# sleveque/control

Measured on NVIDIA B200. Metric: kkt_solve_time, lower is better.
Workload: dtype f64

## Files before the change

### control_b200/_lib.py

```python
import ctypes as C
import os

_HERE = os.path.dirname(os.path.abspath(__file__))
LIB_PATH = os.path.join(_HERE, "lib", "libctl_b200.so")

CTL_LAYOUT_BLOCK_MAJOR, CTL_LAYOUT_TIME_FASTEST = 0, 1
CTL_MAT_M, CTL_MAT_K, CTL_MAT_KT = 0, 1, 2
CTL_KSP_GMRES, CTL_KSP_FGMRES, CTL_KSP_MINRES = 0, 1, 2
CTL_PC_NONE, CTL_PC_BUILTIN, CTL_PC_CALLBACK = 0, 1, 2
CTL_PCMODE_TRIANGULAR, CTL_PCMODE_DIAGONAL = 0, 1
CTL_S0_JACOBI, CTL_S0_CHEBYSHEV, CTL_S0_AMG = 0, 1, 2
CTL_HISTORY_MAX = 1024


class ctl_config(C.Structure):
    _fields_ = [("n", C.c_int32), ("n_t", C.c_int32), ("CN", C.c_int32), ("device", C.c_int32),
                ("tau", C.c_double), ("beta", C.c_double), ("epsilon", C.c_double),
                ("stream", C.c_void_p), ("rank", C.c_int32), ("world", C.c_int32)]


class ctl_pc_options(C.Structure):
    _fields_ = [("mode", C.c_int32), ("solver_0", C.c_int32),
                ("cheb_emin", C.c_double), ("cheb_emax", C.c_double),
                ("cheb_steps", C.c_int32), ("amg_cycles", C.c_int32), ("amg_nu", C.c_int32),
                ("amg_nu_fine", C.c_int32),
                ("amg_max_levels", C.c_int32), ("amg_coarse_max", C.c_int32),
                ("amg_theta", C.c_double), ("amg_lo", C.c_double), ("amg_hi", C.c_double),
                ("amg_acc_lo", C.c_double), ("amg_acc_hi", C.c_double)]


class ctl_krylov_options(C.Structure):
    _fields_ = [("ksp_type", C.c_int32), ("restart", C.c_int32), ("max_it", C.c_int32),
                ("pc", C.c_int32), ("rtol", C.c_double), ("atol", C.c_double),
                ("divtol", C.c_double)]


class ctl_solve_result(C.Structure):
    _fields_ = [("its", C.c_int32), ("reason", C.c_int32), ("n_mult", C.c_int32),
                ("n_pc", C.c_int32), ("rnorm", C.c_double), ("ref_norm", C.c_double),
                ("n_history", C.c_int32), ("history", C.c_double * CTL_HISTORY_MAX),
                ("seconds_total", C.c_double), ("seconds_mult", C.c_double),
                ("seconds_pc", C.c_double)]

# ... 20 lines not shown
    "ctl_set_pattern": (C.c_int, [_H, C.c_void_p, C.c_void_p, C.c_int64]),
    "ctl_set_values": (C.c_int, [_H, C.c_int, C.c_int, C.c_void_p]),
    "ctl_set_bc": (C.c_int, [_H, C.c_void_p, C.c_int32]),
    "ctl_set_block_size": (C.c_int, [_H, C.c_int32]),
    "ctl_assemble": (C.c_int, [_H]),
    "ctl_n_blocks": (C.c_int32, [_H]),
    "ctl_ld": (C.c_int32, [_H]),
    "ctl_n_local": (C.c_int32, [_H]),
    "ctl_row_begin": (C.c_int32, [_H]),
    "ctl_vec_len": (C.c_int64, [_H, C.c_int]),
    "ctl_convert_layout": (C.c_int, [_H, _F64P, C.c_int, _F64P, C.c_int]),
    "ctl_kkt_apply": (C.c_int, [_H, _F64P, _F64P, C.c_int]),
    "ctl_pc_default_options": (C.c_int, [C.POINTER(ctl_pc_options)]),
    "ctl_pc_setup": (C.c_int, [_H, C.POINTER(ctl_pc_options)]),
    "ctl_pc_block_size": (C.c_int32, [_H]),
    "ctl_pc_apply": (C.c_int, [_H, _F64P, _F64P, C.c_int]),
    "ctl_pc_fn": (C.c_int, [_H, _F64P, _F64P, C.c_int]),
    "ctl_set_pc_callback": (C.c_int, [_H, PC_CALLBACK, C.c_void_p]),
    "ctl_krylov_default_options": (C.c_int, [C.POINTER(ctl_krylov_options)]),
    "ctl_solve": (C.c_int, [_H, _F64P, _F64P, C.c_int, C.POINTER(ctl_krylov_options),
                            C.POINTER(ctl_solve_result)]),
    "ctl_solve_host": (C.c_int, [_H, _F64P, _F64P, C.POINTER(ctl_krylov_options),
                                 C.POINTER(ctl_solve_result)]),
    "ctl_kkt_residual_norm": (C.c_int, [_H, _F64P, _F64P, C.c_int, C.POINTER(C.c_double)]),
    "ctl_nonlinear_residual": (C.c_int, [_H, _F64P, _F64P, _F64P, C.c_int, C.POINTER(C.c_double)]),
    "ctl_objective_host": (C.c_int, [_H, _F64P, _F64P, _F64P, C.POINTER(C.c_double)]),
    "ctl_objective": (C.c_int, [_H, _F64P, _F64P, _F64P, C.POINTER(C.c_double)]),
    "ctl_build_rhs": (C.c_int, [_H, _F64P, _F64P, _F64P, _F64P]),
    "ctl_lift_bc": (C.c_int, [_H, _F64P, _F64P, C.c_int]),
    "ctl_amg_num_hierarchies": (C.c_int32, [_H]),
# ... 60 lines not shown
```

### control_b200/csrc/amg.cu

```cuda
#include "amg.cuh"

#include <cstdlib>
#include <stdexcept>

#include "cheb_coefficients.h"

int amg_build_distributed(ctl_handle_s *h, const AmgParams &p, const std::shared_ptr<SellPattern> &fine_pattern,
                          AmgHierarchyDev &H);

static int dev_alloc(ctl_handle_s *h, double **p, size_t n)
{
    CTL_CUDA(cudaMalloc((void **)p, std::max<size_t>(n, 1) * sizeof(double)));
    CTL_CUDA(cudaMemsetAsync(*p, 0, std::max<size_t>(n, 1) * sizeof(double), h->stream));
    return CTL_OK;
}

int amg_level_vectors(ctl_handle_s *h, AmgLevelDev &L, int level)
{
    const size_t nv = (size_t)L.n * L.A.nc;
    CTL_TRY(dev_alloc(h, &L.r, nv));
    CTL_TRY(dev_alloc(h, &L.t0, nv));
    CTL_TRY(dev_alloc(h, &L.t1, nv));
    CTL_TRY(dev_alloc(h, &L.t2, nv));
    if (level > 0) {
// ... 10 lines not shown
    const int64_t nc = H.nc;
    int64_t bytes = 0;
    for (int l = 0; l < nl; ++l) {
        const AmgLevelDev &L = H.dev[l];
        if (l + 1 < nl) {
            const int nu_l = (l == 0 && p.nu_fine > 0) ? p.nu_fine : p.nu;
            bytes += (L.A.bytes_per_pass + (8ll + 32ll * nc) * L.n) * (2 * nu_l);
            bytes += L.P.bytes_per_pass + L.R.bytes_per_pass + 32ll * nc * L.n;
        } else if (L.Ainv) {
            bytes += 8ll * L.n * L.n;
        } else {
            bytes += (L.A.bytes_per_pass + (8ll + 32ll * nc) * L.n) * p.nu;
        }
    }
    return bytes;
}

int amg_build(ctl_handle_s *h, const HostCSR &A0, const AmgParams &p,
              const std::shared_ptr<SellPattern> &fine_pattern, AmgHierarchyDev &H)
{
    H.params = p;
    try {
        if (H.host.empty()) amg_setup_host(A0, p, H.host);
    } catch (const std::exception &e) {
        ctl_set_error(h, e.what());
        return CTL_ERR_STATE;
    }
    const int nl = (int)H.host.size();
    H.dev.assign(nl, AmgLevelDev());
    CTL_CHECK(H.nc == 1 || h->cfg.world == 1, CTL_ERR_ARG, "amg_build: block hierarchies run on one GPU only");
// ... 11 lines not shown
            Ld.A.nc = H.nc;
            CTL_TRY(ctl_upload(h, &Ld.dinv, Lh.dinv.data(), (size_t)Ld.n));
            CTL_TRY(amg_level_vectors(h, Ld, l));
            if (l + 1 < nl) {
                CTL_TRY(sell_from_csr(h, Lh.P, Ld.P));
                CTL_TRY(sell_from_csr(h, Lh.R, Ld.R));
                Ld.P.nc = Ld.R.nc = H.nc;
            } else if (!Lh.Ainv.empty()) {
                CTL_TRY(dense_inverse_upload(h, Lh.Ainv, Ld.n, &Ld.Ainv, &Ld.Ainv_ld));
            } else if (Lh.coarse_inverse) {
                CTL_TRY(dense_inverse_device(h, Lh.A, Lh.coarse_shift, &Ld.Ainv, &Ld.Ainv_ld));
            }
        }
    }
    H.bytes_per_cycle = amg_cycle_bytes(H);
    if (p.acc_lo > 0.0) {
        const size_t nv = (size_t)H.dev[0].n * H.nc;
        CTL_TRY(dev_alloc(h, &H.acc_r, nv));
        CTL_TRY(dev_alloc(h, &H.acc_z, nv));
        CTL_TRY(dev_alloc(h, &H.acc_p, nv));
    }
    return CTL_OK;
}

void amg_free(AmgHierarchyDev &H)
{
    cudaFree(H.acc_r);
    cudaFree(H.acc_z);
    cudaFree(H.acc_p);
    H.acc_r = H.acc_z = H.acc_p = nullptr;
// ... 103 lines not shown

namespace {
__global__ void lincomb3_kernel(double *out, double a, const double *x, double b, const double *__restrict__ y,
                                double c, const double *__restrict__ z, int n)
{
    pdl_sync();
    const int i = blockIdx.x * blockDim.x + threadIdx.x;
    if (i >= n) return;
    double r = c * z[i];
    if (y) r = fma(b, y[i], r);
    if (x) r = fma(a, x[i], r);
    out[i] = r;
}
}

int amg_solve(ctl_handle_s *h, AmgHierarchyDev &H, const double *b, double *x, bool b_exchanged)
{
    const AmgParams &p = H.params;
    AmgLevelDev &L0 = H.dev[0];
    if (L0.pb && !b_exchanged) CTL_TRY(halo_exchange_now(h, L0.pb, b));
    const GVec gb = L0.pb ? GVec(b, halo_ll(L0.pb), halo_idx1(L0.pb)) : GVec(b);
    if (p.acc_lo <= 0.0) {
        for (int c = 0; c < p.cycles; ++c) CTL_TRY(vcycle(h, H, 0, gb, x, c == 0));
        return CTL_OK;
    }
    CTL_CHECK(!L0.px, CTL_ERR_STATE, "amg_solve: accelerated cycles are not available on several GPUs");
    const int n = L0.n * H.nc;
    double scale;
    std::vector<double> om;
    cheb_coefficients(p.acc_lo, p.acc_hi, p.cycles, &scale, om);
    double *buf[2] = {x, H.acc_p};
    auto slot = [&](int k) { return (p.cycles - k) & 1; };
    const int blocks = ceil_div(n, 256);
    CTL_TRY(vcycle(h, H, 0, gb, H.acc_z, true));
// ... 14 lines not shown
```

### control_b200/csrc/amg.cuh

```cuda
#pragma once
#include "amg_setup.h"
#include "sell.cuh"

struct AmgLevelDev {
    int n = 0;
    int n_ghost = 0;
    bool distributed = false;
    double rho = 0.0;
    SellMat A, P, R;
    double *dinv = nullptr;
    double *x = nullptr, *b = nullptr;
    double *r = nullptr, *t0 = nullptr, *t1 = nullptr, *t2 = nullptr;
    double *Ainv = nullptr;
    int Ainv_ld = 0;
    HaloPlan *px = nullptr, *pb = nullptr;
    HaloPlan *pr = nullptr;
    HaloPlan *prep = nullptr;
};

struct AmgHierarchyDev {
    AmgParams params;
    int nc = 1;
    std::vector<AmgLevelHost> host;
    std::vector<AmgLevelDev> dev;
    std::vector<std::shared_ptr<struct HaloSpace>> spaces;
    int64_t bytes_per_cycle = 0;
    double *acc_r = nullptr, *acc_z = nullptr, *acc_p = nullptr;
};

int amg_build(ctl_handle_s *h, const HostCSR &A0, const AmgParams &p,
              const std::shared_ptr<SellPattern> &fine_pattern, AmgHierarchyDev &H);
void amg_free(AmgHierarchyDev &H);
int dense_inverse_device(ctl_handle_s *h, const HostCSR &A, const std::vector<double> &shift, double **Ainv_out, int *lda_out);
int dense_inverse_upload(ctl_handle_s *h, const std::vector<double> &Ainv, int n, double **Ainv_out, int *lda_out);
int amg_solve(ctl_handle_s *h, AmgHierarchyDev &H, const double *b, double *x, bool b_exchanged = false);
```

### control_b200/csrc/amg_setup.h

```cpp
#pragma once
#include <vector>

#include "common.cuh"

enum { AMG_COARSE_INVERSE = 0,
       AMG_COARSE_PINV_CONSTANT = 1,
       AMG_COARSE_SMOOTH = 2 };

struct AmgParams {
    double theta = 0.08;
    double theta_decay = 0.5;
    int max_levels = 10;
    int coarse_max = 2500;
    int nu = 3;
    int nu_fine = 0;
    double lo = 0.25, hi = 1.0;
    int cycles = 3;
    double acc_lo = 0.0, acc_hi = 1.0;
    int coarse = 0;
    int device_inverse = 1;
};

struct AmgLevelHost {
    HostCSR A;
    std::vector<double> dinv;
    double rho = 0.0;
    std::vector<int> agg;
    HostCSR P, R;
    std::vector<double> Ainv;
    int coarse_inverse = 0;
    std::vector<double> coarse_shift;
    bool has_inverse() const { return !Ainv.empty() || coarse_inverse != 0; }
};

// ... 5 lines not shown
```

### control_b200/csrc/pc.cu

```cuda
#include "pc.cuh"

#include <atomic>
#include <chrono>
#include <cstdio>
#include <map>
#include <cmath>
#include <cstdlib>
#include <cstring>
#include <thread>

#include "cheb_coefficients.h"
#include "vec_ops.cuh"

namespace {

void combine_global(ctl_handle_s *h, int level, bool transposed, double w, double m_coef, bool identity,
                    std::vector<double> &out)
{
    const std::vector<int> &ip = h->h_indptr, &ix = h->h_indices;
    const int lv = h->h_K.size() > 1 ? level : 0;
    const std::vector<double> &Kv = h->h_K[lv];
    const std::vector<double> *KTv = h->h_KT.empty() ? nullptr : &h->h_KT[lv];
    out.assign(ix.size(), 0.0);
    for (int r = 0; r < h->n; ++r) {
// ... 291 lines not shown
    o->mode = CTL_PCMODE_TRIANGULAR;
    o->solver_0 = CTL_S0_JACOBI;
    o->cheb_emin = 0.0;
    o->cheb_emax = 0.0;
    o->cheb_steps = 20;
    o->amg_cycles = d.cycles;
    o->amg_nu = d.nu;
    o->amg_nu_fine = d.nu_fine;
    o->amg_max_levels = d.max_levels;
    o->amg_coarse_max = d.coarse_max;
    o->amg_theta = d.theta;
    o->amg_lo = d.lo;
    o->amg_hi = d.hi;
    o->amg_acc_lo = d.acc_lo;
    o->amg_acc_hi = d.acc_hi;
    return CTL_OK;
}

int ctl_amg_setup_probe(const int32_t *indptr, const int32_t *indices, const double *values, int32_t n,
                        const ctl_pc_options *opts, int32_t *n_levels, int32_t *level_n, int64_t *level_nnz,
                        double *level_rho, int32_t *aggregates)
{
    if (!indptr || !indices || !values || n <= 0 || !n_levels) return CTL_ERR_ARG;
    AmgParams p;
    if (opts) {
        p.theta = opts->amg_theta;
        p.max_levels = opts->amg_max_levels;
        p.coarse_max = opts->amg_coarse_max;
        p.nu = opts->amg_nu;
        p.nu_fine = opts->amg_nu_fine;
// ... 46 lines not shown
{
    SetupLap lap;
    CTL_CHECK(h && opts, CTL_ERR_ARG, "ctl_pc_setup: null argument");
    CTL_CHECK(h->assembled, CTL_ERR_STATE, "ctl_pc_setup: ctl_assemble has not been called");
    CTL_CHECK(opts->mode == CTL_PCMODE_TRIANGULAR || opts->mode == CTL_PCMODE_DIAGONAL, CTL_ERR_ARG,
              "ctl_pc_setup: unknown mode");
    CTL_CHECK(opts->solver_0 >= CTL_S0_JACOBI && opts->solver_0 <= CTL_S0_AMG, CTL_ERR_ARG,
              "ctl_pc_setup: unknown solver_0");
    if (opts->solver_0 == CTL_S0_CHEBYSHEV)
        CTL_CHECK(opts->cheb_emax > opts->cheb_emin && opts->cheb_emin > 0 && opts->cheb_steps >= 1, CTL_ERR_ARG,
                  "ctl_pc_setup: Chebyshev needs 0 < e_min < e_max and at least one step");
    CTL_CHECK(opts->amg_cycles >= 1 && opts->amg_nu >= 1 && opts->amg_nu_fine >= 0 && opts->amg_max_levels >= 1,
              CTL_ERR_ARG, "ctl_pc_setup: bad AMG options");
    CTL_CHECK(opts->amg_acc_lo <= 0.0 || opts->amg_acc_hi > opts->amg_acc_lo, CTL_ERR_ARG,
              "ctl_pc_setup: AMG acceleration needs acc_lo < acc_hi");
    if (opts->mode == CTL_PCMODE_DIAGONAL)
        CTL_CHECK(h->cfg.CN && !h->per_level && h->k_symmetric, CTL_ERR_ARG,
                  "ctl_pc_setup: the block-diagonal (MINRES) variant needs CN and a time-independent symmetric K");
    CTL_CHECK(h->cfg.world == 1 || h->comm, CTL_ERR_STATE, "ctl_pc_setup: call ctl_comm_init first (world > 1)");
    CTL_CUDA(cudaSetDevice(h->cfg.device));
    ctl_pc_free(h);
    h->pc = std::make_shared<PcState>();
    PcState &st = *h->pc;
    st.opts = *opts;
    st.amg.theta = opts->amg_theta;
    st.amg.max_levels = opts->amg_max_levels;
    st.amg.coarse_max = opts->amg_coarse_max;
    st.amg.nu = opts->amg_nu;
    st.amg.nu_fine = opts->amg_nu_fine;
    st.amg.lo = opts->amg_lo;
    st.amg.hi = opts->amg_hi;
    st.amg.cycles = opts->amg_cycles;
    st.amg.acc_lo = opts->amg_acc_lo;
    st.amg.acc_hi = opts->amg_acc_hi;
    if (const char *e = getenv("CTL_NO_GRAPH")) st.use_graph = !(e[0] == '1');

    const int N = h->N, nl = h->n_loc, rb = h->row_begin;
    const bool cn = h->cfg.CN != 0;
    const double tau = h->cfg.tau, beta = h->cfg.beta, eps = h->cfg.epsilon;
    if (h->h_KT.empty() && !h->k_symmetric && h->h_tperm.size() != h->h_indices.size()) {
        const std::vector<int> &ip = h->h_indptr, &ix = h->h_indices;
        h->h_tperm.resize(ix.size());
        for (int r = 0; r < h->n; ++r)
            for (int k = ip[r]; k < ip[r + 1]; ++k) {
                const int c = ix[k];
                const int *b = ix.data() + ip[c], *e = ix.data() + ip[c + 1];
                h->h_tperm[k] = (int)(std::lower_bound(b, e, r) - ix.data());
            }
    }
// ... 251 lines not shown
    std::copy(A.indptr.begin(), A.indptr.end(), indptr);
    std::copy(A.indices.begin(), A.indices.end(), indices);
    std::copy(A.values.begin(), A.values.end(), values);
    return CTL_OK;
}

int ctl_amg_get_aggregates(ctl_handle h, int32_t hi, int32_t lvl, int32_t *agg)
{
    AMG_LEVEL(h, hi, lvl);
    std::copy(L.agg.begin(), L.agg.end(), agg);
    return CTL_OK;
}

int32_t ctl_pc_block_size(ctl_handle h) { return (h && h->pc && h->pc->ready) ? h->pc->bs : -1; }

int ctl_amg_solve(ctl_handle h, int32_t hi, const double *b, double *x)
{
    CTL_CHECK(h && h->pc && hi >= 0 && hi < (int)h->pc->hier.size() && b && x, CTL_ERR_ARG, "ctl_amg_solve: bad argument");
    CTL_CHECK(h->pc->hier[hi].nc != 2 || (((uintptr_t)b | (uintptr_t)x) & 15) == 0, CTL_ERR_ARG,
              "ctl_amg_solve: a block-size-2 hierarchy needs 16-byte aligned vectors");
    CTL_CUDA(cudaSetDevice(h->cfg.device));
    CTL_TRY(halo_epoch_begin(h));
    CTL_TRY(amg_solve(h, h->pc->hier[hi], b, x, false));
    return ctl_comm_check(h);
}

int ctl_time_amg(ctl_handle h, int32_t hi, int reps, int flush_l2, double *out)
{
    CTL_CHECK(h && h->pc && hi >= 0 && hi < (int)h->pc->hier.size() && out && reps > 0, CTL_ERR_ARG,
              "ctl_time_amg: bad argument");
// ... 73 lines not shown
```

### control_b200/csrc/sell.cu

```cuda
#include <algorithm>
#include <cstdlib>
#include <cstring>
#include <type_traits>

#include "sell.cuh"

SellPattern::~SellPattern()
{
    cudaFree(sp);
    cudaFree(cols);
    cudaFree(dcol);
}

void sell_free(SellMat &m)
{
    cudaFree(m.vals);
    cudaFree(m.vcode);
    cudaFree(m.vdict);
    cudaFree(m.code);
    cudaFree(m.dict);
    cudaFree(m.sp4);
    cudaFree(m.stab);
    cudaFree(m.csr_ptr);
    cudaFree(m.csr_cols);
// ... 298 lines not shown
    if constexpr (NC == 2) {
        *reinterpret_cast<double2 *>(out + 2 * row) = make_double2(v.c[0], v.c[1]);
    } else {
#pragma unroll
        for (int k = 0; k < NC; ++k) out[NC * row + k] = v.c[k];
    }
}
template <int NC>
__device__ __forceinline__ vec_t<NC> gat(const DVec &v, int c, unsigned seq_hi, const HaloCtx &ctx)
{
    if constexpr (NC == 1) return dvec_get(v, c, seq_hi, ctx);
    else return ld_node<NC>(v.x, c);
}

template <typename G, typename G0, typename PRE>
__device__ __forceinline__ auto sell_row_dot_stencil(const MatView &A, int row, G g, G0 g_own, PRE pre)
{
    const int s = row >> 5, lane = row & 31;
    const int4 s0 = pre_ld(A.sp4 + s);
    const int first = s << 5;
    const bool spec = A.ps_w > 0 && first + A.ps_dmin >= 0 && first + 31 + A.ps_dmax < A.n_own;
    pdl_wait();
    pre();
    using R = decltype(g(0));
    R acc{};
    if (spec) {
        R xv[8];
#pragma unroll
        for (int j = 0; j < 8; ++j) xv[j] = (j < A.ps_w) ? g_own(row + A.ps_delta[j]) : R{};
        if (s0.z == A.ps_off) {
#pragma unroll
            for (int j = 0; j < 8; ++j)
                if (j < A.ps_w) acc = vfma(A.ps_v[j], xv[j], acc);
            if (A.ps_w > 8) {
// ... 31 lines not shown
            for (int j = 0; j < SC; ++j) xv[j] = (k0 + j < s0.y) ? g(row + d[j]) : R{};
#pragma unroll
            for (int j = 0; j < SC; ++j)
                if (k0 + j < s0.y) acc = vfma(__ldg(&st[k0 + j].v), xv[j], acc);
        }
        return acc;
    }
    const int end = s0.x + 32 * s0.y;
    const uint16_t *code = reinterpret_cast<const uint16_t *>(A.code);
#pragma unroll 1
    for (int p = s0.x + lane; p < end; p += 32) {
        const DictEnt e = sf_dict(A.dict, __ldg(code + p));
        acc = vfma(e.v, g(row + e.delta), acc);
    }
    return acc;
}

template <int FMT, bool STREAM, typename G, typename G0, typename PRE>
__device__ __forceinline__ auto sell_row_dot(const MatView &A, int row, G g, G0 g_own, PRE pre)
{
    if (FMT == FMT_STENCIL) return sell_row_dot_stencil(A, row, g, g_own, pre);
    const int s = row >> 5, lane = row & 31;
    const int2 s0 = pre_ld(A.sp + s);
    const int end = pre_ld(reinterpret_cast<const int *>(A.sp + s + 1));
    using R = decltype(g(0));
    R acc{};
    auto chunk = [&](int p0, auto first) {
        constexpr bool PRE = decltype(first)::value;
        SfRaw raw[SC];
#pragma unroll
// ... 215 lines not shown
{
    const unsigned hi = kernel_prologue(ctx);
    run_rows<1, BS>(A.n_rows, push, hi, out, [&](int row) {
        const double di = pre_ld(dinv.x + row);
        vec_t<NC> bi{};
        const vec_t<NC> ax = sell_row_dot<FMT, STREAM>(
            A, row,
            [&](int c) {
                if constexpr (GH) return s * dvec_get(dinv, c, hi, ctx) * dvec_get(b, c, hi, ctx);
                else return s * __ldg(dinv.x + c) * ld_node<NC>(b.x, c);
            },
            [&](int c) { return s * __ldg(dinv.x + c) * ld_node<NC>(b.x, c); }, [&] { bi = ld_node<NC>(b.x, row); });
        const vec_t<NC> p1 = s * di * bi;
        return wgt * p1 + (wgt * s) * di * (bi - ax);
    });
}

template <int NC>
__global__ void __launch_bounds__(ST) sell_spmv2_kernel(const MatView A1, const MatView A2, const DVec x1, const DVec x2,
                                                       const DVec x3, double *y, double alpha, double beta,
                                                       const HaloCtx ctx, const HaloPush push)
{
    const unsigned hi = kernel_prologue(ctx);
    run_rows<1>(A1.n_rows, push, hi, y, [&](int row) {
        vec_t<NC> acc1;
        if (x2.x) acc1 = sell_row_dot_rt(A1, row, [&](int c) { return gat<NC>(x1, c, hi, ctx) + gat<NC>(x2, c, hi, ctx); });
        else acc1 = sell_row_dot_rt(A1, row, [&](int c) { return gat<NC>(x1, c, hi, ctx); });
        vec_t<NC> acc2{};
        if (x3.x) acc2 = sell_row_dot_rt(A2, row, [&](int c) { return gat<NC>(x3, c, hi, ctx); });
        return alpha * acc1 + beta * acc2;
// ... 333 lines not shown
    const DVec d1 = dvec(x1, V1), d2 = dvec(x2, V1), d3 = dvec(x3, V2);
    const HaloCtx ctx = halo_ctx(h);
    if (A1.nc == 2) pdl_launch(h, grid, ST, sell_spmv2_kernel<2>, V1, V2, d1, d2, d3, y, alpha, beta, ctx, push);
    else if (A1.nc == 3) pdl_launch(h, grid, ST, sell_spmv2_kernel<3>, V1, V2, d1, d2, d3, y, alpha, beta, ctx, push);
    else pdl_launch(h, grid, ST, sell_spmv2_kernel<1>, V1, V2, d1, d2, d3, y, alpha, beta, ctx, push);
    h->launches++;
    CTL_CUDA(cudaGetLastError());
    return CTL_OK;
}

int vec_copy_n(ctl_handle_s *h, double *dst, const double *src, int n)
{
    CTL_CUDA(cudaMemcpyAsync(dst, src, (size_t)n * sizeof(double), cudaMemcpyDeviceToDevice, h->stream));
    return CTL_OK;
}
```

### control_b200/csrc/sell.cuh

```cuda
#pragma once
#include <memory>

#include "common.cuh"
#include "halo.cuh"
#include "sell_format.h"

struct SellPattern {
    int n_rows = 0, n_cols = 0, n_slices = 0;
    int64_t n_stored = 0, nnz = 0;
    int2 *sp = nullptr;
    int *cols = nullptr;
    uint16_t *dcol = nullptr;
    SfSellLayout host;
    ~SellPattern();
};

struct SellMat {
    std::shared_ptr<SellPattern> pat;
    int fmt = FMT_F64;
    bool stream = false;
    int n_own = 0;
    int nc = 1;
    int64_t bytes_per_pass = 0;
    double *vals = nullptr;
// ... 42 lines not shown
};

int sell_spmv(ctl_handle_s *h, const SellMat &A, const GVec &x, double *y, const double *b, int mode,
              const HaloPush &push = HaloPush());
int sell_cheb_step(ctl_handle_s *h, const SellMat &A, const double *dinv, const double *b, const double *p_prev,
                   const GVec &p_cur, double *out, double a, double bq, double c, double prev_scale = 0.0,
                   const HaloPush &push = HaloPush());
int sell_cheb_first2(ctl_handle_s *h, const SellMat &A, const GVec &dinv, const GVec &b, double *out, double s, double w,
                     const HaloPush &push = HaloPush());
int vec_dinv_scale(ctl_handle_s *h, const double *dinv, const double *b, double *out, double c, int n,
                   const HaloPush &push = HaloPush(), int nc = 1);
int dense_gemv(ctl_handle_s *h, const double *Ainv, const double *b, double *y, int n, int lda, int nc = 1);
int sell_spmv2(ctl_handle_s *h, const SellMat &A1, const SellMat &A2, const GVec &x1, const GVec &x2, const GVec &x3,
               double *y, double alpha, double beta, const HaloPush &push = HaloPush());
int vec_copy_n(ctl_handle_s *h, double *dst, const double *src, int n);
```

### control_b200/system.py

```python
import ctypes as C

import numpy as np
import torch

from . import _lib as L

__all__ = ["MultiBlockSystem", "KSPInfo", "csr_arrays"]

_KSP_TYPES = {"gmres": L.CTL_KSP_GMRES, "fgmres": L.CTL_KSP_FGMRES, "minres": L.CTL_KSP_MINRES}

_error_flag = [False]


def csr_arrays(A):
    if isinstance(A, (tuple, list)) and len(A) == 3:
        indptr, indices, data = A
    else:
        A = A.tocsr()
        if not A.has_sorted_indices:
            A = A.sorted_indices()
        indptr, indices, data = A.indptr, A.indices, A.data
    return (np.ascontiguousarray(indptr, dtype=np.int32),
            np.ascontiguousarray(indices, dtype=np.int32),
            np.ascontiguousarray(data, dtype=np.float64))
# ... 203 lines not shown
        o = L.ctl_pc_options()
        self._check(self._lib.ctl_pc_default_options(C.byref(o)))
        o.mode = {"triangular": L.CTL_PCMODE_TRIANGULAR, "diagonal": L.CTL_PCMODE_DIAGONAL}[mode]
        if Multigrid:
            o.solver_0 = L.CTL_S0_AMG
        elif lambda_v_bounds is not None:
            o.solver_0 = L.CTL_S0_CHEBYSHEV
            o.cheb_emin, o.cheb_emax = float(lambda_v_bounds[0]), float(lambda_v_bounds[1])
        else:
            o.solver_0 = L.CTL_S0_JACOBI
        o.cheb_steps = int(cheb_steps)
        for key, field in (("cycles", "amg_cycles"), ("nu", "amg_nu"), ("nu_fine", "amg_nu_fine"),
                           ("max_levels", "amg_max_levels"),
                           ("coarse_max", "amg_coarse_max"), ("theta", "amg_theta"),
                           ("lo", "amg_lo"), ("hi", "amg_hi"), ("acc_lo", "amg_acc_lo"),
                           ("acc_hi", "amg_acc_hi")):
            if key in amg:
                setattr(o, field, amg.pop(key))
        if amg:
            raise TypeError(f"unknown AMG options {sorted(amg)}")
        self._check(self._lib.ctl_pc_setup(self._h, C.byref(o)))
        self._pc_ready = True
        self._pc_opts = o

    @property
    def pc_block_size(self):
        return int(self._lib.ctl_pc_block_size(self._h))

    def pc_apply(self, b_dev, u_dev=None, layout=L.CTL_LAYOUT_BLOCK_MAJOR, raw=False):
        if u_dev is None:
            u_dev = torch.zeros_like(b_dev)
        fn = self._lib.ctl_pc_fn if raw else self._lib.ctl_pc_apply
        self._call(fn, b_dev.data_ptr(), u_dev.data_ptr(), layout)
        return u_dev

    def pc_fn(self):
        def pc_fn(u_0, u_1, b_0, b_1):
            u = self.pc_apply(self.to_device(b_0, b_1), raw=True)
            r0, r1 = self.to_host_blocks(u)
            np.copyto(_as_host_f64(u_0).reshape(r0.shape), r0)
            np.copyto(_as_host_f64(u_1).reshape(r1.shape), r1)
        return pc_fn
# ... 271 lines not shown
```

### include/ctl_b200.h

```cpp
#ifndef CTL_B200_H
#define CTL_B200_H

#include <stdint.h>

#ifdef __cplusplus
extern "C" {
#endif

typedef struct ctl_handle_s *ctl_handle;

enum { CTL_OK = 0, CTL_ERR_ARG = -1, CTL_ERR_CUDA = -2, CTL_ERR_STATE = -3, CTL_ERR_NCCL = -4,
       CTL_ERR_CALLBACK = -5 };

enum { CTL_LAYOUT_BLOCK_MAJOR = 0, CTL_LAYOUT_TIME_FASTEST = 1 };

enum { CTL_MAT_M = 0, CTL_MAT_K = 1, CTL_MAT_KT = 2 };

enum { CTL_KSP_GMRES = 0, CTL_KSP_FGMRES = 1, CTL_KSP_MINRES = 2 };

enum { CTL_PC_NONE = 0,
       CTL_PC_BUILTIN = 1,
       CTL_PC_CALLBACK = 2 };

enum { CTL_PCMODE_TRIANGULAR = 0,
// ... 21 lines not shown
} ctl_config;

typedef struct {
    int32_t mode;
    int32_t solver_0;
    double cheb_emin, cheb_emax;
    int32_t cheb_steps;
    int32_t amg_cycles;
    int32_t amg_nu;
    int32_t amg_nu_fine;
    int32_t amg_max_levels;
    int32_t amg_coarse_max;
    double amg_theta;
    double amg_lo, amg_hi;
    double amg_acc_lo, amg_acc_hi;
} ctl_pc_options;

typedef struct {
    int32_t ksp_type;
    int32_t restart;
    int32_t max_it;
    int32_t pc;
    double rtol, atol;
    double divtol;
} ctl_krylov_options;

#define CTL_HISTORY_MAX 1024
typedef struct {
    int32_t its;
    int32_t reason;
// ... 21 lines not shown
int ctl_assemble(ctl_handle h);

int32_t ctl_n_blocks(ctl_handle h);
int32_t ctl_ld(ctl_handle h);
int32_t ctl_n_local(ctl_handle h);
int32_t ctl_row_begin(ctl_handle h);
int64_t ctl_vec_len(ctl_handle h, int layout);
int ctl_convert_layout(ctl_handle h, const double *src, int src_layout, double *dst,
                       int dst_layout);

int ctl_kkt_apply(ctl_handle h, const double *x, double *y, int layout);

int ctl_pc_default_options(ctl_pc_options *opts);
int ctl_pc_setup(ctl_handle h, const ctl_pc_options *opts);
int32_t ctl_pc_block_size(ctl_handle h);
int ctl_pc_apply(ctl_handle h, const double *b, double *u, int layout);
int ctl_pc_fn(ctl_handle h, const double *b, double *u, int layout);
int ctl_set_pc_callback(ctl_handle h, ctl_pc_callback fn, void *user);

int ctl_krylov_default_options(ctl_krylov_options *opts);
int ctl_solve(ctl_handle h, const double *b, double *u, int layout,
              const ctl_krylov_options *opts, ctl_solve_result *result);
int ctl_solve_host(ctl_handle h, const double *b_host, double *u_host,
                   const ctl_krylov_options *opts, ctl_solve_result *result);

int ctl_kkt_residual_norm(ctl_handle h, const double *b, const double *x, int layout,
                          double *out);
int ctl_nonlinear_residual(ctl_handle h, const double *b, const double *x, double *r, int layout,
                           double *norm_host);
int ctl_objective_host(ctl_handle h, const double *v_host, const double *zeta_host,
// ... 62 lines not shown
```

Measured before the change: 1.198.

## Fuse multiple fine-level Chebyshev smoothing steps into one shared-memory tiled kernel

Adds a temporal-blocking kernel that keeps a tile of the fine-level iterate plus a halo of k*band rows in shared memory and applies up to k Chebyshev/residual steps per launch. The plan derives band width and tile size from the stencil pattern, SM count and opt-in shared memory. The AMG solve switches to this fused path when conditions hold (single device, stencil format, single component, no acceleration), which is on by default (-1). The aim is fewer kernel launches and less global memory traffic per smoother sweep, at the cost of redundant halo computation and one block per SM.

```diff
diff --git a/control_b200/_lib.py b/control_b200/_lib.py
--- a/control_b200/_lib.py
+++ b/control_b200/_lib.py
@@ -26,7 +26,7 @@
                 ("amg_nu_fine", C.c_int32),
                 ("amg_max_levels", C.c_int32), ("amg_coarse_max", C.c_int32),
                 ("amg_theta", C.c_double), ("amg_lo", C.c_double), ("amg_hi", C.c_double),
-                ("amg_acc_lo", C.c_double), ("amg_acc_hi", C.c_double)]
+                ("amg_acc_lo", C.c_double), ("amg_acc_hi", C.c_double), ("amg_fine_fusion", C.c_int32)]
 
 
 class ctl_krylov_options(C.Structure):
@@ -77,6 +77,8 @@
     "ctl_pc_default_options": (C.c_int, [C.POINTER(ctl_pc_options)]),
     "ctl_pc_setup": (C.c_int, [_H, C.POINTER(ctl_pc_options)]),
     "ctl_pc_block_size": (C.c_int32, [_H]),
+    "ctl_pc_fine_fusion": (C.c_int32, [_H]),
+    "ctl_fine_fusion_plan": (C.c_int, [C.c_int32, C.c_int32, C.c_int32, C.c_int32, C.c_int32, _I32P]),
     "ctl_pc_apply": (C.c_int, [_H, _F64P, _F64P, C.c_int]),
     "ctl_pc_fn": (C.c_int, [_H, _F64P, _F64P, C.c_int]),
     "ctl_set_pc_callback": (C.c_int, [_H, PC_CALLBACK, C.c_void_p]),
diff --git a/control_b200/csrc/amg.cu b/control_b200/csrc/amg.cu
--- a/control_b200/csrc/amg.cu
+++ b/control_b200/csrc/amg.cu
@@ -48,6 +48,29 @@
         }
     }
     return bytes;
+}
+
+static int fine_fusion_setup(ctl_handle_s *h, AmgHierarchyDev &H)
+{
+    H.ff = FfPlan();
+    const AmgParams &p = H.params;
+    const int nu0 = p.nu_fine > 0 ? p.nu_fine : p.nu;
+    if (p.fine_fusion == 0 || h->cfg.world > 1 || H.nc != 1 || p.acc_lo > 0.0 || H.dev.size() < 2 || nu0 < 2) return CTL_OK;
+    const AmgLevelDev &L = H.dev[0];
+    if (L.A.lanes || L.A.fmt != FMT_STENCIL || L.px || L.pb) return CTL_OK;
+    const SfSellLayout &lay = L.A.pat->host;
+    int band = 0;
+    for (int s = 0; s < lay.n_slices; ++s)
+        for (int64_t q = lay.sp[s].x; q < lay.sp[s + 1].x; ++q) {
+            const int row = 32 * s + (int)((q - lay.sp[s].x) & 31);
+            if (row < L.n) band = std::max(band, std::abs(lay.cols[q] - row));
+        }
+    int dev = 0, n_sm = 0, smem = 0;
+    CTL_CUDA(cudaGetDevice(&dev));
+    CTL_CUDA(cudaDeviceGetAttribute(&n_sm, cudaDevAttrMultiProcessorCount, dev));
+    CTL_CUDA(cudaDeviceGetAttribute(&smem, cudaDevAttrMaxSharedMemoryPerBlockOptin, dev));
+    H.ff = fine_fusion_plan(L.n, band, n_sm, smem, p.fine_fusion > 0 ? p.fine_fusion : 0);
+    return sell_fused_prepare(h, H.ff);
 }
 
 int amg_build(ctl_handle_s *h, const HostCSR &A0, const AmgParams &p,
@@ -89,6 +112,7 @@
         }
     }
     H.bytes_per_cycle = amg_cycle_bytes(H);
+    CTL_TRY(fine_fusion_setup(h, H));
     if (p.acc_lo > 0.0) {
         const size_t nv = (size_t)H.dev[0].n * H.nc;
         CTL_TRY(dev_alloc(h, &H.acc_r, nv));
@@ -222,10 +246,102 @@
 }
 }
 
+static int amg_solve_fused(ctl_handle_s *h, AmgHierarchyDev &H, const double *b, double *x)
+{
+    const AmgParams &p = H.params;
+    AmgLevelDev &L = H.dev[0];
+    AmgLevelDev &C = H.dev[1];
+    const int nu = p.nu_fine > 0 ? p.nu_fine : p.nu;
+    double scale;
+    std::vector<double> om;
+    cheb_coefficients(p.lo * L.rho, p.hi * L.rho, nu, &scale, om);
+    auto step = [&](int k, bool zero) {
+        FfOp o;
+        o.kind = FF_CHEB;
+        if (k == 1) {
+            o.a = 0.0;
+            o.bq = 1.0;
+            o.c = scale;
+        } else {
+            const double w = om[k - 2];
+            o.a = 1.0 - w;
+            o.bq = w;
+            o.c = w * scale;
+            if (zero && k == 3) o.prev_scale = scale;
+        }
+        return o;
+    };
+    double *pool[5] = {x, L.t0, L.t1, L.t2, L.r};
+    auto run_chain = [&](const std::vector<FfOp> &ops, const double *cur_in, double **res) -> int {
+        const int k = H.ff.k, n_ops = (int)ops.size();
+        const double *in_cur = cur_in, *in_prev = nullptr;
+        for (int g0 = 0; g0 < n_ops; g0 += k) {
+            FfGroup g;
+            g.n_ops = std::min(k, n_ops - g0);
+            for (int j = 0; j < g.n_ops; ++j) g.op[j] = ops[g0 + j];
+            g.cur_in = in_cur;
+            g.prev_in = in_prev;
+            const bool final = g0 + g.n_ops == n_ops;
+            const FfOp &next = final ? ops[0] : ops[g0 + g.n_ops];
+            const bool need_prev = !final && next.kind == FF_CHEB && next.prev_scale == 0.0 && next.a != 0.0;
+            std::vector<double *> free_;
+            for (double *v : pool)
+                if (v != in_cur && v != in_prev && v != x) free_.push_back(v);
+            if (final) {
+                g.cur_out = x;
+                if (ops.back().kind == FF_RES) {
+                    g.res_out = free_[0];
+                    *res = g.res_out;
+                }
+            } else {
+                g.cur_out = free_[0];
+                g.prev_out = need_prev ? free_[1] : nullptr;
+            }
+            CTL_CHECK(final || g.op[g.n_ops - 1].kind != FF_RES, CTL_ERR_STATE, "amg_solve: residual inside a chain");
+            CTL_TRY(sell_fused_group(h, L.A, H.ff, L.dinv, b, g));
+            in_cur = g.cur_out;
+            in_prev = g.prev_out;
+        }
+        return CTL_OK;
+    };
+    FfOp res;
+    res.kind = FF_RES;
+    std::vector<FfOp> chain;
+    const double *chain_in = nullptr;
+    for (int c = 0; c < p.cycles; ++c) {
+        if (c == 0) {
+            FfOp f2;
+            f2.kind = FF_FIRST2;
+            f2.c = scale;
+            f2.bq = om[0];
+            chain.push_back(f2);
+            for (int k = 3; k <= nu; ++k) chain.push_back(step(k, true));
+        } else {
+            for (int k = 1; k <= nu; ++k) chain.push_back(step(k, false));
+        }
+        chain.push_back(res);
+        double *r = nullptr;
+        CTL_TRY(run_chain(chain, chain_in, &r));
+        CTL_TRY(sell_spmv(h, L.R, GVec(r), C.b, nullptr, SELL_ASSIGN));
+        CTL_TRY(vcycle(h, H, 1, GVec(C.b), C.x, true));
+        CTL_TRY(sell_spmv(h, L.P, GVec(C.x), L.t2, x, SELL_BPLUS));
+        chain.clear();
+        for (int k = 1; k <= nu; ++k) chain.push_back(step(k, false));
+        chain_in = L.t2;
+        if (c + 1 == p.cycles) {
+            double *none = nullptr;
+            CTL_TRY(run_chain(chain, chain_in, &none));
+        }
+    }
+    CTL_CUDA(cudaGetLastError());
+    return CTL_OK;
+}
+
 int amg_solve(ctl_handle_s *h, AmgHierarchyDev &H, const double *b, double *x, bool b_exchanged)
 {
     const AmgParams &p = H.params;
     AmgLevelDev &L0 = H.dev[0];
+    if (H.ff.k > 0) return amg_solve_fused(h, H, b, x);
     if (L0.pb && !b_exchanged) CTL_TRY(halo_exchange_now(h, L0.pb, b));
     const GVec gb = L0.pb ? GVec(b, halo_ll(L0.pb), halo_idx1(L0.pb)) : GVec(b);
     if (p.acc_lo <= 0.0) {
diff --git a/control_b200/csrc/amg.cuh b/control_b200/csrc/amg.cuh
--- a/control_b200/csrc/amg.cuh
+++ b/control_b200/csrc/amg.cuh
@@ -26,6 +26,7 @@
     std::vector<std::shared_ptr<struct HaloSpace>> spaces;
     int64_t bytes_per_cycle = 0;
     double *acc_r = nullptr, *acc_z = nullptr, *acc_p = nullptr;
+    FfPlan ff;
 };
 
 int amg_build(ctl_handle_s *h, const HostCSR &A0, const AmgParams &p,
diff --git a/control_b200/csrc/amg_setup.h b/control_b200/csrc/amg_setup.h
--- a/control_b200/csrc/amg_setup.h
+++ b/control_b200/csrc/amg_setup.h
@@ -18,6 +18,7 @@
     int cycles = 3;
     double acc_lo = 0.0, acc_hi = 1.0;
     int coarse = 0;
+    int fine_fusion = 0;
     int device_inverse = 1;
 };
 
diff --git a/control_b200/csrc/pc.cu b/control_b200/csrc/pc.cu
--- a/control_b200/csrc/pc.cu
+++ b/control_b200/csrc/pc.cu
@@ -329,6 +329,7 @@
     o->amg_hi = d.hi;
     o->amg_acc_lo = d.acc_lo;
     o->amg_acc_hi = d.acc_hi;
+    o->amg_fine_fusion = -1;
     return CTL_OK;
 }
 
@@ -405,6 +406,7 @@
               CTL_ERR_ARG, "ctl_pc_setup: bad AMG options");
     CTL_CHECK(opts->amg_acc_lo <= 0.0 || opts->amg_acc_hi > opts->amg_acc_lo, CTL_ERR_ARG,
               "ctl_pc_setup: AMG acceleration needs acc_lo < acc_hi");
+    CTL_CHECK(opts->amg_fine_fusion >= -1, CTL_ERR_ARG, "ctl_pc_setup: amg_fine_fusion must be -1, 0 or positive");
     if (opts->mode == CTL_PCMODE_DIAGONAL)
         CTL_CHECK(h->cfg.CN && !h->per_level && h->k_symmetric, CTL_ERR_ARG,
                   "ctl_pc_setup: the block-diagonal (MINRES) variant needs CN and a time-independent symmetric K");
@@ -424,6 +426,7 @@
     st.amg.cycles = opts->amg_cycles;
     st.amg.acc_lo = opts->amg_acc_lo;
     st.amg.acc_hi = opts->amg_acc_hi;
+    st.amg.fine_fusion = opts->amg_fine_fusion;
     if (const char *e = getenv("CTL_NO_GRAPH")) st.use_graph = !(e[0] == '1');
 
     const int N = h->N, nl = h->n_loc, rb = h->row_begin;
@@ -705,6 +708,23 @@
 
 int32_t ctl_pc_block_size(ctl_handle h) { return (h && h->pc && h->pc->ready) ? h->pc->bs : -1; }
 
+int32_t ctl_pc_fine_fusion(ctl_handle h)
+{
+    if (!(h && h->pc && h->pc->ready)) return -1;
+    return h->pc->hier.empty() ? 0 : h->pc->hier[0].ff.k;
+}
+
+int ctl_fine_fusion_plan(int32_t n, int32_t band, int32_t n_sm, int32_t smem_max, int32_t k_cap, int32_t *out)
+{
+    if (!out || n < 0 || band < 0 || n_sm <= 0 || smem_max <= 0 || k_cap < 0) return CTL_ERR_ARG;
+    const FfPlan p = fine_fusion_plan(n, band, n_sm, smem_max, k_cap);
+    out[0] = p.k;
+    out[1] = p.tile;
+    out[2] = p.tiles;
+    out[3] = p.smem;
+    return CTL_OK;
+}
+
 int ctl_amg_solve(ctl_handle h, int32_t hi, const double *b, double *x)
 {
     CTL_CHECK(h && h->pc && hi >= 0 && hi < (int)h->pc->hier.size() && b && x, CTL_ERR_ARG, "ctl_amg_solve: bad argument");
diff --git a/control_b200/csrc/sell.cu b/control_b200/csrc/sell.cu
--- a/control_b200/csrc/sell.cu
+++ b/control_b200/csrc/sell.cu
@@ -336,10 +336,9 @@
 }
 
 template <typename G, typename G0, typename PRE>
-__device__ __forceinline__ auto sell_row_dot_stencil(const MatView &A, int row, G g, G0 g_own, PRE pre)
+__device__ __forceinline__ auto sell_row_dot_stencil_s0(const MatView &A, int row, const int4 s0, G g, G0 g_own, PRE pre)
 {
     const int s = row >> 5, lane = row & 31;
-    const int4 s0 = pre_ld(A.sp4 + s);
     const int first = s << 5;
     const bool spec = A.ps_w > 0 && first + A.ps_dmin >= 0 && first + 31 + A.ps_dmax < A.n_own;
     pdl_wait();
@@ -401,6 +400,12 @@
         acc = vfma(e.v, g(row + e.delta), acc);
     }
     return acc;
+}
+
+template <typename G, typename G0, typename PRE>
+__device__ __forceinline__ auto sell_row_dot_stencil(const MatView &A, int row, G g, G0 g_own, PRE pre)
+{
+    return sell_row_dot_stencil_s0(A, row, pre_ld(A.sp4 + (row >> 5)), g, g_own, pre);
 }
 
 template <int FMT, bool STREAM, typename G, typename G0, typename PRE>
@@ -646,6 +651,106 @@
         const vec_t<NC> p1 = s * di * bi;
         return wgt * p1 + (wgt * s) * di * (bi - ax);
     });
+}
+
+constexpr int FF_BS = 512;
+constexpr int FF_U = 4;
+constexpr int FF_S = 8;
+
+template <int BS>
+__global__ void __launch_bounds__(BS, 1) sell_fused_kernel(const MatView A, const DVec dinv, const double *b, const FfGroup g,
+                                                          int tile, int band)
+{
+    extern __shared__ double ff_buf[];
+    pdl_trigger();
+    const int n = A.n_rows, k = g.n_ops;
+    const int r0 = blockIdx.x * tile, r1 = min(n, r0 + tile);
+    const int lo0 = max(0, r0 - k * band), hi0 = min(n, r1 + k * band);
+    double *cur = ff_buf, *prv = ff_buf + (tile + 2 * k * band);
+    pdl_wait();
+    const bool first2 = g.op[0].kind == FF_FIRST2;
+    const double s1 = g.op[0].c;
+    for (int i0 = lo0 + (int)threadIdx.x; i0 < hi0; i0 += FF_S * BS) {
+        double v[FF_S], w[FF_S];
+#pragma unroll
+        for (int u = 0; u < FF_S; ++u) {
+            const int i = min(i0 + u * BS, hi0 - 1);
+            if (first2) {
+                v[u] = s1 * __ldg(dinv.x + i) * b[i];
+            } else {
+                v[u] = g.cur_in[i];
+                if (g.prev_in) w[u] = g.prev_in[i];
+            }
+        }
+#pragma unroll
+        for (int u = 0; u < FF_S; ++u) {
+            const int i = i0 + u * BS;
+            if (i < hi0) {
+                cur[i - lo0] = v[u];
+                if (!first2 && g.prev_in) prv[i - lo0] = w[u];
+            }
+        }
+    }
+    __syncthreads();
+    for (int j = 0; j < k; ++j) {
+        const FfOp o = g.op[j];
+        const bool last = j == k - 1;
+        const int ext = (k - 1 - j) * band;
+        const int lo = max(0, r0 - ext), hi = min(n, r1 + ext);
+        const double *cb = cur - lo0;
+        double *pb = prv - lo0;
+        auto gs = [&](int c) { return cb[c]; };
+        for (int base = (lo & ~31) + (int)threadIdx.x; base < hi; base += FF_U * BS) {
+            int4 s0[FF_U];
+            double di[FF_U], bi[FF_U];
+#pragma unroll
+            for (int u = 0; u < FF_U; ++u) {
+                const int row = min(max(base + u * BS, lo), hi - 1);
+                s0[u] = pre_ld(A.sp4 + (row >> 5));
+                di[u] = __ldg(dinv.x + row);
+                bi[u] = b[row];
+            }
+#pragma unroll
+            for (int u = 0; u < FF_U; ++u) {
+                const int row = base + u * BS;
+                if (row < lo || row >= hi) continue;
+                double v;
+                if (o.kind == FF_FIRST2) {
+                    const double s = o.c, wgt = o.bq;
+                    const double ax = sell_row_dot_stencil_s0(A, row, s0[u], gs, gs, [] {});
+                    const double p1 = s * di[u] * bi[u];
+                    v = wgt * p1 + (wgt * s) * di[u] * (bi[u] - ax);
+                } else if (o.kind == FF_CHEB) {
+                    const double a = o.a, bq = o.bq, c = o.c, prev_scale = o.prev_scale;
+                    const double pc = cb[row];
+                    double pp{};
+                    if (prev_scale == 0.0 && a != 0.0) pp = pb[row];
+                    const double ax = sell_row_dot_stencil_s0(A, row, s0[u], gs, gs, [] {});
+                    double r = bq * pc + c * di[u] * (bi[u] - ax);
+                    if (prev_scale != 0.0) r = vfma(a, prev_scale * di[u] * bi[u], r);
+                    else if (a != 0.0) r = vfma(a, pp, r);
+                    v = r;
+                } else {
+                    v = bi[u] - sell_row_dot_stencil_s0(A, row, s0[u], gs, gs, [] {});
+                }
+                if (!last) {
+                    pb[row] = v;
+                } else if (o.kind == FF_RES) {
+                    g.res_out[row] = v;
+                    if (g.cur_out) g.cur_out[row] = cb[row];
+                } else {
+                    g.cur_out[row] = v;
+                    if (g.prev_out) g.prev_out[row] = cb[row];
+                }
+            }
+        }
+        if (!last) {
+            __syncthreads();
+            double *t = cur;
+            cur = prv;
+            prv = t;
+        }
+    }
 }
 
 template <int NC>
@@ -1009,3 +1114,60 @@
     CTL_CUDA(cudaMemcpyAsync(dst, src, (size_t)n * sizeof(double), cudaMemcpyDeviceToDevice, h->stream));
     return CTL_OK;
 }
+
+FfPlan fine_fusion_plan(int n, int band, int n_sm, int smem_max, int k_cap)
+{
+    FfPlan p;
+    p.band = band;
+    if (n <= 0 || band <= 0 || n_sm <= 0) return p;
+    int64_t T = std::max<int64_t>(ceil_div((int64_t)n, n_sm), 4ll * band);
+    T = std::min<int64_t>(ceil_div(T, 32) * 32, ceil_div((int64_t)n, 32) * 32);
+    const int64_t cap = smem_max / 16;
+    int64_t k = cap > T ? (cap - T) / (2ll * band) : 0;
+    k = std::min<int64_t>({k, T / band, (int64_t)FF_KMAX});
+    if (k_cap > 0) k = std::min<int64_t>(k, k_cap);
+    if (k < 2) return p;
+    p.k = (int)k;
+    p.tile = (int)T;
+    p.tiles = (int)ceil_div((int64_t)n, T);
+    p.smem = (int)(16 * (T + 2 * k * band));
+    return p;
+}
+
+int sell_fused_prepare(ctl_handle_s *h, const FfPlan &p)
+{
+    if (p.k == 0) return CTL_OK;
+    CTL_CUDA(cudaFuncSetAttribute(sell_fused_kernel<FF_BS>, cudaFuncAttributeMaxDynamicSharedMemorySize, p.smem));
+    return CTL_OK;
+}
+
+int sell_fused_group(ctl_handle_s *h, const SellMat &A, const FfPlan &p, const double *dinv, const double *b,
+                     const FfGroup &g)
+{
+    CTL_CHECK(A.lanes == 0 && A.fmt == FMT_STENCIL && A.nc == 1, CTL_ERR_STATE,
+              "sell_fused_group: a one-component STENCIL matrix only");
+    CTL_CHECK(g.n_ops >= 1 && g.n_ops <= p.k && p.k > 0, CTL_ERR_STATE, "sell_fused_group: more ops than the plan");
+    CTL_CHECK(g.op[0].kind == FF_FIRST2 || g.cur_in, CTL_ERR_STATE, "sell_fused_group: no input iterate");
+    const FfOp &e = g.op[g.n_ops - 1];
+    CTL_CHECK(e.kind == FF_RES ? g.res_out != nullptr : g.cur_out != nullptr, CTL_ERR_STATE, "sell_fused_group: no output");
+    for (const double *o : {(const double *)g.cur_out, (const double *)g.prev_out, (const double *)g.res_out})
+        CTL_CHECK(!o || (o != g.cur_in && o != g.prev_in && o != b), CTL_ERR_STATE,
+                  "sell_fused_group: an output aliases an input");
+    const MatView V = A.view();
+    DVec dd{};
+    dd.x = dinv;
+    dd.n_own = V.n_own;
+    cudaLaunchConfig_t cfg{};
+    cfg.gridDim = dim3(p.tiles);
+    cfg.blockDim = dim3(FF_BS);
+    cfg.dynamicSmemBytes = p.smem;
+    cfg.stream = h->stream;
+    cudaLaunchAttribute at;
+    at.id = cudaLaunchAttributeProgrammaticStreamSerialization;
+    at.val.programmaticStreamSerializationAllowed = 1;
+    cfg.attrs = &at;
+    cfg.numAttrs = h->use_pdl ? 1 : 0;
+    CTL_CUDA(cudaLaunchKernelEx(&cfg, sell_fused_kernel<FF_BS>, V, dd, b, g, p.tile, p.band));
+    h->launches++;
+    return CTL_OK;
+}
diff --git a/control_b200/csrc/sell.cuh b/control_b200/csrc/sell.cuh
--- a/control_b200/csrc/sell.cuh
+++ b/control_b200/csrc/sell.cuh
@@ -80,3 +80,25 @@
 int sell_spmv2(ctl_handle_s *h, const SellMat &A1, const SellMat &A2, const GVec &x1, const GVec &x2, const GVec &x3,
                double *y, double alpha, double beta, const HaloPush &push = HaloPush());
 int vec_copy_n(ctl_handle_s *h, double *dst, const double *src, int n);
+
+constexpr int FF_KMAX = 8;
+enum { FF_FIRST2 = 0, FF_CHEB = 1, FF_RES = 2 };
+struct FfOp {
+    int kind = FF_CHEB;
+    double a = 0.0, bq = 0.0, c = 0.0, prev_scale = 0.0;
+};
+struct FfGroup {
+    int n_ops = 0;
+    FfOp op[FF_KMAX];
+    const double *cur_in = nullptr, *prev_in = nullptr;
+    double *cur_out = nullptr;
+    double *prev_out = nullptr;
+    double *res_out = nullptr;
+};
+struct FfPlan {
+    int band = 0, k = 0, tile = 0, tiles = 0, smem = 0;
+};
+FfPlan fine_fusion_plan(int n, int band, int n_sm, int smem_max, int k_cap);
+int sell_fused_prepare(ctl_handle_s *h, const FfPlan &p);
+int sell_fused_group(ctl_handle_s *h, const SellMat &A, const FfPlan &p, const double *dinv, const double *b,
+                     const FfGroup &g);
diff --git a/control_b200/system.py b/control_b200/system.py
--- a/control_b200/system.py
+++ b/control_b200/system.py
@@ -241,7 +241,7 @@
                            ("max_levels", "amg_max_levels"),
                            ("coarse_max", "amg_coarse_max"), ("theta", "amg_theta"),
                            ("lo", "amg_lo"), ("hi", "amg_hi"), ("acc_lo", "amg_acc_lo"),
-                           ("acc_hi", "amg_acc_hi")):
+                           ("acc_hi", "amg_acc_hi"), ("fine_fusion", "amg_fine_fusion")):
             if key in amg:
                 setattr(o, field, amg.pop(key))
         if amg:
@@ -253,6 +253,10 @@
     @property
     def pc_block_size(self):
         return int(self._lib.ctl_pc_block_size(self._h))
+
+    @property
+    def pc_fine_fusion(self):
+        return int(self._lib.ctl_pc_fine_fusion(self._h))
 
     def pc_apply(self, b_dev, u_dev=None, layout=L.CTL_LAYOUT_BLOCK_MAJOR, raw=False):
         if u_dev is None:
diff --git a/include/ctl_b200.h b/include/ctl_b200.h
--- a/include/ctl_b200.h
+++ b/include/ctl_b200.h
@@ -59,6 +59,7 @@
     double amg_theta;
     double amg_lo, amg_hi;
     double amg_acc_lo, amg_acc_hi;
+    int32_t amg_fine_fusion;
 } ctl_pc_options;
 
 typedef struct {
@@ -110,6 +111,8 @@
 int ctl_pc_default_options(ctl_pc_options *opts);
 int ctl_pc_setup(ctl_handle h, const ctl_pc_options *opts);
 int32_t ctl_pc_block_size(ctl_handle h);
+int32_t ctl_pc_fine_fusion(ctl_handle h);
+int ctl_fine_fusion_plan(int32_t n, int32_t band, int32_t n_sm, int32_t smem_max, int32_t k_cap, int32_t *out);
 int ctl_pc_apply(ctl_handle h, const double *b, double *u, int layout);
 int ctl_pc_fn(ctl_handle h, const double *b, double *u, int layout);
 int ctl_set_pc_callback(ctl_handle h, ctl_pc_callback fn, void *user);
diff --git a/prof_ff.py b/prof_ff.py
--- /dev/null
+++ b/prof_ff.py
@@ -0,0 +1,32 @@
+import sys, os, json, ctypes as C
+import numpy as np, torch
+sys.path.insert(0, os.path.dirname(os.path.abspath(__file__)))
+from synthetic import problems
+from control_b200 import MultiBlockSystem
+from torch.profiler import profile, ProfilerActivity
+q = problems.heat_problem(1024, 4, True)
+s = MultiBlockSystem(q["M"], q["K"], n_t=4, beta=q["beta"], CN=True, time_interval=q["time_interval"], bc_dofs=q["bdofs"], device=0)
+lib = s._lib
+b = torch.tensor(np.random.default_rng(0).standard_normal(s.n), device="cuda:0", dtype=torch.float64)
+x = torch.zeros_like(b)
+for ff in (0, -1, 2, 0, -1):
+    s.setup_preconditioner(lambda_v_bounds=q["lambda_v_bounds"], mode="diagonal", cycles=2, nu=4, fine_fusion=ff)
+    for _ in range(30): s._call(lib.ctl_amg_solve, 0, b.data_ptr(), x.data_ptr())
+    torch.cuda.synchronize()
+    e0, e1 = torch.cuda.Event(enable_timing=True), torch.cuda.Event(enable_timing=True)
+    e0.record()
+    for _ in range(300): s._call(lib.ctl_amg_solve, 0, b.data_ptr(), x.data_ptr())
+    e1.record(); torch.cuda.synchronize()
+    us = e0.elapsed_time(e1) * 1e3 / 300
+    with profile(activities=[ProfilerActivity.CUDA]) as p:
+        for _ in range(20): s._call(lib.ctl_amg_solve, 0, b.data_ptr(), x.data_ptr())
+        torch.cuda.synchronize()
+    agg = {}
+    for ev in p.events():
+        if ev.device_type.name == "CUDA":
+            k = ev.name[:90]
+            a = agg.setdefault(k, [0, 0.0]); a[0] += 1; a[1] += ev.device_time
+    rows = sorted(agg.items(), key=lambda kv: -kv[1][1])
+    print(json.dumps({"ff": ff, "k": s.pc_fine_fusion, "inner_us": round(us, 1)}), flush=True)
+    for k, (c, t) in rows[:14]:
+        print(f"   {c/20:5.1f}/solve  {t/c:7.2f} us  {t/20:7.1f} us/solve  {k}", flush=True)
```

New measurement: 1.914, median of 6. 59.8% more time.
